# AliaksandrSiarohin/wc-gan

Hardware: AMD Instinct MI355X
Metric: images/sec G+D step, CIFAR-10 ResNet-SN+WC, batch 64 (higher is better)
Workload: dtype f32; 1 GPU; CIFAR-10 ResNet SN uncond + WC (scripts/cifar10_resnet_sn_uncond.sh), batch 64/GPU, training_ratio 5, generator_batch_multiple 2; parallelism=dp1, wc_statistics=per-replica, launch=hipgraph

## Files before the change

wc_gan_amd/csrc/wc_conv.hip:

```cpp
#include "wc_common.h"
#include "../../include/wc_hip.h"
#include <stdlib.h>
#include <string.h>


namespace {

constexpr int kMaxTaps = 16, kMaxPhase = 4;

struct ConvArgs {
    const _Float16* xhi; const _Float16* xlo;
    const _Float16* zero;
    const char* wimg;
    const float* xscale; const float* wscale;
    const float* bias;
    float* y;
    int N, H, W, Hin, Win, Cin, Cout, in_stride, ntaps, nphase, Hout, Wout, out_stride, relu;
    unsigned magHW, shHW, magW, shW;
    int ksplit; float* partial;
    signed char dy[kMaxPhase][kMaxTaps], dx[kMaxPhase][kMaxTaps];
    signed char offy[kMaxPhase], offx[kMaxPhase];
};

__device__ __forceinline__ void lds_dma16(const void* g, unsigned lds)
{
    unsigned keep;
    asm volatile("s_mov_b32 %0, m0\n\ts_mov_b32 m0, %2\n\ts_nop 0\n\tglobal_load_lds_dwordx4 %1, off\n\ts_mov_b32 m0, %0"
                 : "=&s"(keep) : "v"(g), "s"(lds) : "memory");
}

template <int MB, int NB, bool KS>
__device__ __forceinline__ void conv_f16x3_body(const ConvArgs& a, const unsigned bx, const unsigned by, const unsigned bz)
{
    extern __shared__ __attribute__((aligned(16))) char smem[];
    constexpr int TM = 64 * MB, TN = 64 * NB;
    constexpr int A_BYTES = 2 * MB * 4 * 1024, B_BYTES = 2 * NB * 4 * 1024, STAGE = A_BYTES + B_BYTES;
    constexpr int AQ = (2 * MB) / 4;
    static_assert(AQ >= 1, "MB >= 2");

    const int tid = threadIdx.x, lane = tid & 63;
    const int wave = __builtin_amdgcn_readfirstlane(tid >> 6);
    const int wm = wave >> 1, wn = wave & 1;
    const int ntn = a.Cout / TN;
    const int phase = by / ntn, nt = by - phase * ntn;
    const unsigned m0 = bx * TM;
    const unsigned HW = a.H * a.W;
    const int koff = (lane >> 5) * 8;

    int gy[AQ], gx[AQ];
    unsigned gpix[AQ];
    #pragma unroll
    for (int q = 0; q < AQ; ++q) {
        const unsigned m = m0 + (wave * AQ + q) * 32 + (lane & 31);
        const unsigned n = __umulhi(m, a.magHW) >> a.shHW, rem = m - n * HW;
        const unsigned yy = __umulhi(rem, a.magW) >> a.shW, xx = rem - yy * a.W;
        gy[q] = yy * a.in_stride; gx[q] = xx * a.in_stride; gpix[q] = n * (a.Hin * a.Win);
    }
    const unsigned lds0 = (unsigned)(size_t)((__attribute__((address_space(3))) char*)smem);
    const int nchunk = a.Cin >> 5;
    const int iters = a.ntaps * nchunk;
    const int nblk_all = a.Cout >> 5;

    auto issue = [&](int it, int stage) {
        const int tap = it / nchunk, ch = it - tap * nchunk;
        const int dy = a.dy[phase][tap], dx = a.dx[phase][tap];
        const unsigned sbase = __builtin_amdgcn_readfirstlane(lds0 + stage * STAGE);
        #pragma unroll
        for (int q = 0; q < AQ; ++q) {
            const int iy = gy[q] + dy, ix = gx[q] + dx;
            const bool ok = (unsigned)iy < (unsigned)a.Hin && (unsigned)ix < (unsigned)a.Win;
            const int64_t e = ((int64_t)(gpix[q] + iy * a.Win + ix)) * a.Cin + ch * 32 + koff;
            #pragma unroll
            for (int s = 0; s < 2; ++s) {
                const _Float16* ph = ok ? a.xhi + e + s * 16 : a.zero + koff;
                const _Float16* pl = ok ? a.xlo + e + s * 16 : a.zero + koff;
                const unsigned l = sbase + (((wave * AQ + q) * 2 + s) * 2) * 1024;
                lds_dma16(ph, l);
                lds_dma16(pl, l + 1024);
            }
        }
        const char* wsrc = a.wimg + ((((int64_t)(phase * a.ntaps + tap) * nchunk + ch) * nblk_all + nt * 2 * NB) << 12);
        #pragma unroll
        for (int c = 0; c < 2 * NB; ++c) {
            const int idx = wave * 2 * NB + c;
            lds_dma16(wsrc + idx * 1024 + lane * 16, sbase + A_BYTES + idx * 1024);
        }
    };

    f32x16 acc[MB][NB];
    #pragma unroll
    for (int i = 0; i < MB; ++i)
        #pragma unroll
        for (int j = 0; j < NB; ++j)
            #pragma unroll
            for (int r = 0; r < 16; ++r) acc[i][j][r] = 0.f;

    const int it0 = KS ? (int)bz * iters / a.ksplit : 0, it1 = KS ? ((int)bz + 1) * iters / a.ksplit : iters;
    constexpr int NA = AQ * 4, ND = NA + 2 * NB, HALF = ND / 2, PER = 3 * MB * NB, GAP = PER / HALF;
    static_assert(PER % HALF == 0, "DMAs spread evenly");
    int tabv = 0;
    if (lane < a.ntaps) tabv = (a.dy[phase][lane] & 0xff) | ((a.dx[phase][lane] & 0xff) << 8);
    const char* pa[AQ][2];
    int pstep[AQ];
    const char* pw;
    unsigned sb_next = 0;
    auto prep = [&](int it, int stage) {
        const int tap = it / nchunk, ch = it - tap * nchunk;
        const int p = __builtin_amdgcn_readlane(tabv, tap);
        const int dy = (signed char)(p & 0xff), dx = (signed char)((p >> 8) & 0xff);
        #pragma unroll
        for (int q = 0; q < AQ; ++q) {
            const int iy = gy[q] + dy, ix = gx[q] + dx;
            const bool ok = (unsigned)iy < (unsigned)a.Hin && (unsigned)ix < (unsigned)a.Win;
            const int64_t e = ((int64_t)(gpix[q] + iy * a.Win + ix)) * a.Cin + ch * 32 + koff;
            pa[q][0] = reinterpret_cast<const char*>(ok ? a.xhi + e : a.zero + koff);
            pa[q][1] = reinterpret_cast<const char*>(ok ? a.xlo + e : a.zero + koff);
            pstep[q] = ok ? 32 : 0;
        }
        pw = a.wimg + ((((int64_t)(phase * a.ntaps + tap) * nchunk + ch) * nblk_all + nt * 2 * NB) << 12) + wave * (2 * NB * 1024) + lane * 16;
        sb_next = __builtin_amdgcn_readfirstlane(lds0 + stage * STAGE);
    };
    auto dma = [&](int d) {
        if (d < NA) {
            const int q = d >> 2, ks = (d >> 1) & 1, pl = d & 1;
            lds_dma16(pa[q][pl] + ks * pstep[q], sb_next + (((wave * AQ + q) * 2 + ks) * 2 + pl) * 1024);
        } else {
            const int c = d - NA;
            lds_dma16(pw + c * 1024, sb_next + A_BYTES + (wave * 2 * NB + c) * 1024);
        }
    };
    f16x8 fa[2][MB][2], fb[2][NB][2];
    auto frags = [&](int stage, int ks) {
        const char* sa = smem + stage * STAGE;
        const char* sb = sa + A_BYTES;
        #pragma unroll
        for (int i = 0; i < MB; ++i) {
            const char* p = sa + (((wm * MB + i) * 2 + ks) * 2) * 1024 + lane * 16;
            fa[ks][i][0] = *reinterpret_cast<const f16x8*>(p);
            fa[ks][i][1] = *reinterpret_cast<const f16x8*>(p + 1024);
        }
        #pragma unroll
        for (int j = 0; j < NB; ++j) {
            const char* p = sb + (((wn * NB + j) * 2 + ks) * 2) * 1024 + lane * 16;
            fb[ks][j][0] = *reinterpret_cast<const f16x8*>(p);
            fb[ks][j][1] = *reinterpret_cast<const f16x8*>(p + 1024);
        }
    };
    prep(it0, 0);
    #pragma unroll
    for (int d = 0; d < ND; ++d) dma(d);
    for (int it = it0; it < it1; ++it) {
        const int stage = (it - it0) & 1;
        __builtin_amdgcn_s_waitcnt(0x0F70);
        __syncthreads();
        frags(stage, 0);
        prep(it + 1 < it1 ? it + 1 : it, stage ^ 1);
        __builtin_amdgcn_sched_barrier(0);
        #pragma unroll
        for (int ks = 0; ks < 2; ++ks) {
            #pragma unroll
            for (int g = 0; g < PER; ++g) {
                const int prod = g / (MB * NB), i = (g / NB) % MB, j = g % NB;
                acc[i][j] = __builtin_amdgcn_mfma_f32_32x32x16_f16(fa[ks][i][prod == 0 ? 1 : 0], fb[ks][j][prod == 1 ? 1 : 0], acc[i][j], 0, 0, 0);
                if ((g + 1) % GAP == 0) {
                    dma(ks * HALF + g / GAP);
                    __builtin_amdgcn_sched_barrier(0);
                }
                if (ks == 0 && g == PER / 2) {
                    frags(stage, 1);
                    __builtin_amdgcn_sched_barrier(0);
                }
            }
        }
    }
    __builtin_amdgcn_s_waitcnt(0x0F70);
    const float inv = 1.0f / (a.xscale[0] * a.wscale[0]);
    const int oy0 = a.offy[phase], ox0 = a.offx[phase];
    float bj[NB];
    #pragma unroll
    for (int j = 0; j < NB; ++j) bj[j] = a.bias ? a.bias[nt * TN + (wn * NB + j) * 32 + (lane & 31)] : 0.f;
    #pragma unroll
    for (int i = 0; i < MB; ++i) {
        #pragma unroll
        for (int r = 0; r < 16; ++r) {
            const unsigned row = (r & 3) + 8 * (r >> 2) + 4 * (lane >> 5);
            const unsigned m = m0 + (wm * MB + i) * 32 + row;
            const unsigned n = __umulhi(m, a.magHW) >> a.shHW, rem = m - n * HW;
            const unsigned yy = __umulhi(rem, a.magW) >> a.shW, xx = rem - yy * a.W;
            const int64_t opix = ((int64_t)n * a.Hout + (yy * a.out_stride + oy0)) * a.Wout + (xx * a.out_stride + ox0);
            const int64_t oe = opix * a.Cout + nt * TN + wn * NB * 32 + (lane & 31);
            if (KS) {
                float* o = a.partial + (int64_t)bz * ((int64_t)a.N * a.Hout * a.Wout * a.Cout) + oe;
                #pragma unroll
                for (int j = 0; j < NB; ++j) o[j * 32] = acc[i][j][r];
            } else {
                float* o = a.y + oe;
                #pragma unroll
                for (int j = 0; j < NB; ++j) {
                    float v = acc[i][j][r] * inv + bj[j];
                    if (a.relu) v = fmaxf(v, 0.f);
                    o[j * 32] = v;
                }
            }
        }
    }
}

template <int MB, int NB, bool KS>
__global__ __launch_bounds__(256) void conv_f16x3_kernel(ConvArgs a) { conv_f16x3_body<MB, NB, KS>(a, blockIdx.x, blockIdx.y, blockIdx.z); }

struct KsplitReduceArgs {
    const float* partial; int ksplit; int64_t n4; int cout;
    const float* xscale; const float* wscale; const float* bias; int relu; float* y;
};

__device__ __forceinline__ void conv_ksplit_reduce_body(const float* __restrict__ partial, int ksplit, int64_t n4, int cout,
                                                        const float* __restrict__ xscale, const float* __restrict__ wscale,
                                                        const float* __restrict__ bias, int relu, float* __restrict__ y,
                                                        const unsigned bid, const unsigned nblocks, const float* __restrict__ res = nullptr)
{
    const float inv = 1.0f / (xscale[0] * wscale[0]);
    for (int64_t i = (int64_t)bid * 256 + threadIdx.x; i < n4; i += (int64_t)nblocks * 256) {
        f32x4 v = *reinterpret_cast<const f32x4*>(partial + 4 * i);
        int z = 1;
        for (; z + 3 < ksplit; z += 4) {
            f32x4 t[4];
            #pragma unroll
            for (int u = 0; u < 4; ++u) t[u] = *reinterpret_cast<const f32x4*>(partial + 4 * ((z + u) * n4 + i));
            #pragma unroll
            for (int u = 0; u < 4; ++u) v += t[u];
        }
        for (; z < ksplit; ++z) v += *reinterpret_cast<const f32x4*>(partial + 4 * (z * n4 + i));
        v = v * inv;
        if (bias) v += *reinterpret_cast<const f32x4*>(bias + (4 * i) % cout);
        if (relu) { v[0] = fmaxf(v[0], 0.f); v[1] = fmaxf(v[1], 0.f); v[2] = fmaxf(v[2], 0.f); v[3] = fmaxf(v[3], 0.f); }
        if (res) {
            const f32x4 r = *reinterpret_cast<const f32x4*>(res + 4 * i);
            #pragma unroll
            for (int j = 0; j < 4; ++j) v[j] = __fadd_rn(v[j], r[j]);
        }
        *reinterpret_cast<f32x4*>(y + 4 * i) = v;
    }
}

__global__ __launch_bounds__(256) void conv_ksplit_reduce_kernel(const float* __restrict__ partial, int ksplit, int64_t n4, int cout,
                                                                 const float* __restrict__ xscale, const float* __restrict__ wscale,
                                                                 const float* __restrict__ bias, int relu, float* __restrict__ y)
{
    conv_ksplit_reduce_body(partial, ksplit, n4, cout, xscale, wscale, bias, relu, y, blockIdx.x, gridDim.x);
}

__global__ __launch_bounds__(256) void conv_ksplit_reduce_res_kernel(const float* __restrict__ partial, int ksplit, int64_t n4, int cout,
                                                                     const float* __restrict__ xscale, const float* __restrict__ wscale,
                                                                     const float* __restrict__ bias, const float* __restrict__ res,
                                                                     float* __restrict__ y)
{
    conv_ksplit_reduce_body(partial, ksplit, n4, cout, xscale, wscale, bias, 0, y, blockIdx.x, gridDim.x, res);
}

__device__ __forceinline__ f32x4 split_act(f32x4 v, int relu, float slope)
{
    if (relu == 1) { v[0] = fmaxf(v[0], 0.f); v[1] = fmaxf(v[1], 0.f); v[2] = fmaxf(v[2], 0.f); v[3] = fmaxf(v[3], 0.f); }
    else if (relu == 2) {
        #pragma unroll
        for (int j = 0; j < 4; ++j) v[j] = v[j] > 0.f ? v[j] : slope * v[j];
    }
    return v;
}

constexpr int kAmaxBlocks = 512;

__global__ __launch_bounds__(256) void conv_absmax_kernel(const float* __restrict__ x, int64_t n4, int64_t n, float* __restrict__ partial,
                                                          float* __restrict__ colsum = nullptr, int c4n = 0, float leaky = -1.f)
{
    __shared__ float red[4];
    __shared__ f32x4 red4[256];
    float m = 0.f;
    f32x4 cs = {0.f, 0.f, 0.f, 0.f};
    for (int64_t i = blockIdx.x * 256 + threadIdx.x; i < n4; i += (int64_t)gridDim.x * 256) {
        const f32x4 v = *reinterpret_cast<const f32x4*>(x + 4 * i);
        const f32x4 u = leaky >= 0.f ? split_act(v, 2, leaky) : v;
        m = fmaxf(fmaxf(m, fabsf(u[0])), fmaxf(fabsf(u[1]), fmaxf(fabsf(u[2]), fabsf(u[3]))));
        cs += v;
    }
    if (blockIdx.x == 0 && threadIdx.x == 0) for (int64_t i = 4 * n4; i < n; ++i) m = fmaxf(m, fabsf(x[i]));
    #pragma unroll
    for (int o = 32; o > 0; o >>= 1) m = fmaxf(m, __shfl_xor(m, o));
    if ((threadIdx.x & 63) == 0) red[threadIdx.x >> 6] = m;
    if (colsum) red4[threadIdx.x] = cs;
    __syncthreads();
    if (threadIdx.x == 0) partial[blockIdx.x] = fmaxf(fmaxf(red[0], red[1]), fmaxf(red[2], red[3]));
    if (colsum && (int)threadIdx.x < c4n) {
        f32x4 t = red4[threadIdx.x];
        for (int p = threadIdx.x + c4n; p < 256; p += c4n) t += red4[p];
        *reinterpret_cast<f32x4*>(colsum + (int64_t)blockIdx.x * 4 * c4n + 4 * threadIdx.x) = t;
    }
}

__device__ __forceinline__ float scale_of(const float* __restrict__ partial, float mul = 1.0f, int count = kAmaxBlocks)
{
    float amax = 0.f;
    for (int i = threadIdx.x & 63; i < count; i += 64) amax = fmaxf(amax, partial[i]);
    #pragma unroll
    for (int o = 32; o > 0; o >>= 1) amax = fmaxf(amax, __shfl_xor(amax, o));
    amax *= mul;
    if (!(amax > 0.f) || !(amax < 3.0e38f)) return 1.0f;
    int e;
    (void)frexpf(amax, &e);
    return ldexpf(1.0f, 14 - e);
}

__global__ __launch_bounds__(256) void conv_leaky_bwd_kernel(float* __restrict__ dx, const float* __restrict__ x, int64_t n4, float slope)
{
    for (int64_t i = blockIdx.x * 256 + threadIdx.x; i < n4; i += (int64_t)gridDim.x * 256) {
        f32x4 g = *reinterpret_cast<const f32x4*>(dx + 4 * i);
        const f32x4 v = *reinterpret_cast<const f32x4*>(x + 4 * i);
        #pragma unroll
        for (int j = 0; j < 4; ++j) g[j] = v[j] > 0.f ? g[j] : slope * g[j];
        *reinterpret_cast<f32x4*>(dx + 4 * i) = g;
    }
}

template <bool DOWN>
__global__ __launch_bounds__(256) void conv_block_dx_kernel(const float* __restrict__ dx1, const float* __restrict__ x,
                                                            const float* __restrict__ other, int64_t n4, int c4, int W, int H,
                                                            float* __restrict__ out)
{
    for (int64_t i = (int64_t)blockIdx.x * 256 + threadIdx.x; i < n4; i += (int64_t)gridDim.x * 256) {
// ... 676 lines not shown

__global__ __launch_bounds__(256) void conv_wrw_narrow_reduce_kernel(const float* __restrict__ partial, int nparts, int Cin, int ks, int nrow,
                                                                     float* __restrict__ dw, int64_t sk, int64_t sn, int64_t sr, int64_t ss,
                                                                     float* __restrict__ db, int Cout)
{
    __shared__ float red[8][32];
    const int el = threadIdx.x & 31, pg = threadIdx.x >> 5;
    const int e = blockIdx.x * 32 + el;
    const float* p = partial + (int64_t)blockIdx.y * nparts * 4096 + e;
    float sum = 0.f;
    int z = pg;
    for (; z + 8 * 15 < nparts; z += 8 * 16) {
        float v[16];
#pragma unroll
        for (int u = 0; u < 16; ++u) v[u] = p[(int64_t)(z + 8 * u) * 4096];
#pragma unroll
        for (int u = 0; u < 16; ++u) sum += v[u];
    }
    for (; z < nparts; z += 8) sum += p[(int64_t)z * 4096];
    red[pg][el] = sum;
    __syncthreads();
    if (pg != 0) return;
#pragma unroll
    for (int g = 1; g < 8; ++g) sum += red[g][el];
    const int q = e >> 10, r = (e >> 6) & 15, ln = e & 63;
    const int row = (r & 3) + 8 * (r >> 2) + 4 * (ln >> 5);
    const int o = blockIdx.y * 128 + 4 * (ln & 31) + q;
    if (o >= Cout) return;
    if (row < nrow) {
        const int tap = row / Cin, c = row - tap * Cin;
        dw[c * sk + o * sn + (tap / ks) * sr + (tap % ks) * ss] = sum;
    } else if (row == nrow && db) db[o] = sum;
}

struct NarrowFwdArgs {
    const float* x; const float* w; const float* bias; float* y;
    int N, H, W, Cin, Cout, ks, nrow, relu;
    int64_t sk, sn, sr, ss;
    unsigned magHW, shHW, magW, shW;
    int64_t M; int ntiles, tiles_per_wave;
    signed char tdy[32], tdx[32], tch[32], tr[32], ts[32];
};

constexpr int kNarrowLd = 32 * 2 + 4;
constexpr int kNarrowNQ = 2;
template <int KS>
__global__ __launch_bounds__(256, 2) void conv_fwd_narrow_kernel(NarrowFwdArgs a)
{
    __shared__ __attribute__((aligned(16))) float nf_tile[4 * 32 * kNarrowLd];
    const int tid = threadIdx.x, lane = tid & 63;
    const int wave = __builtin_amdgcn_readfirstlane(tid >> 6);
    const int i = lane & 31, k = lane >> 5;
    const int grp = blockIdx.y;
    __shared__ float nf_w[32][32 * kNarrowNQ];
    __shared__ int nf_tab[32][2];
#pragma unroll
    for (int j = 0; j < 8; ++j) {
        const int m = wave + 4 * j;
        const int kind = m < a.nrow ? 0 : (m == a.nrow ? 1 : 2);
        const int o = grp * (32 * kNarrowNQ) + lane;
        float v = 0.f;
        if (kind == 0) v = a.w[a.tch[m] * a.sk + o * a.sn + a.tr[m] * a.sr + a.ts[m] * a.ss];
        else if (kind == 1) v = a.bias ? a.bias[o] : 0.f;
        nf_w[m][lane] = v;
        if (lane == 0) {
            const int dy = a.tdy[m], dx = a.tdx[m];
            nf_tab[m][0] = (dy & 0xff) | ((dx & 0xff) << 8) | (kind << 16);
            nf_tab[m][1] = (dy * a.W + dx) * a.Cin + a.tch[m];
        }
    }
    __syncthreads();
    int dyx[KS], off[KS]; float bw[KS][kNarrowNQ];
#pragma unroll
    for (int s = 0; s < KS; ++s) {
        const int m = 2 * s + k;
        dyx[s] = nf_tab[m][0];
        off[s] = nf_tab[m][1];
#pragma unroll
        for (int q = 0; q < kNarrowNQ; ++q) bw[s][q] = nf_w[m][q * 32 + i];
    }
    const unsigned HW = (unsigned)(a.H * a.W);
    const int t0 = (blockIdx.x * 4 + wave) * a.tiles_per_wave;
    int t1 = t0 + a.tiles_per_wave;
    if (t1 > a.ntiles) t1 = a.ntiles;
    auto gather = [&](int t, float (&av)[KS]) __attribute__((always_inline)) {
        const int64_t p = (int64_t)t * 32 + i;
        const unsigned pc = (unsigned)(p < a.M ? p : a.M - 1);
        const unsigned n = __umulhi(pc, a.magHW) >> a.shHW, rem = pc - n * HW;
        const unsigned yy = __umulhi(rem, a.magW) >> a.shW, xx = rem - yy * a.W;
        const int pb = (int)pc * a.Cin;
#pragma unroll
        for (int s = 0; s < KS; ++s) {
            const int dy = (signed char)(dyx[s] & 0xff), dx = (signed char)((dyx[s] >> 8) & 0xff), kind = dyx[s] >> 16;
            const bool inb = kind == 0 && (unsigned)((int)yy + dy) < (unsigned)a.H && (unsigned)((int)xx + dx) < (unsigned)a.W;
            const float xv = a.x[inb ? pb + off[s] : 0];
            av[s] = inb ? xv : (kind == 1 ? 1.f : 0.f);
        }
    };
    float av[KS], an[KS];
    if (t0 < t1) gather(t0, av);
    for (int t = t0; t < t1; ++t) {
        if (t + 1 < t1) gather(t + 1, an);
        f32x16 acc[kNarrowNQ];
#pragma unroll
        for (int q = 0; q < kNarrowNQ; ++q)
#pragma unroll
            for (int r = 0; r < 16; ++r) acc[q][r] = 0.f;
#pragma unroll
        for (int s = 0; s < KS; ++s)
#pragma unroll
            for (int q = 0; q < kNarrowNQ; ++q) acc[q] = __builtin_amdgcn_mfma_f32_32x32x2f32(av[s], bw[s][q], acc[q], 0, 0, 0);
        float* tl = nf_tile + wave * (32 * kNarrowLd);
#pragma unroll
        for (int r = 0; r < 16; ++r) {
            const int row = (r & 3) + 8 * (r >> 2) + 4 * k;
#pragma unroll
            for (int q = 0; q < kNarrowNQ; ++q) {
                float v = acc[q][r];
                if (a.relu) v = fmaxf(v, 0.f);
                tl[row * kNarrowLd + q * 32 + i] = v;
            }
        }
        __builtin_amdgcn_s_waitcnt(0xc07f);
#pragma unroll
        for (int j = 0; j < 8; ++j) {
            const int row = 4 * j + (lane >> 4);
            const int64_t pr = (int64_t)t * 32 + row;
            const f32x4 v = *reinterpret_cast<const f32x4*>(tl + row * kNarrowLd + 4 * (lane & 15));
            if (pr < a.M) *reinterpret_cast<f32x4*>(a.y + pr * a.Cout + grp * (32 * kNarrowNQ) + 4 * (lane & 15)) = v;
        }
#pragma unroll
        for (int s = 0; s < KS; ++s) av[s] = an[s];
    }
}

void magic_u31(unsigned d, unsigned* mag, unsigned* sh)
{
    unsigned s = 0;
    while ((1u << s) < d) ++s;
    const unsigned long long num = 1ull << (31 + s);
    *mag = (unsigned)((num + d - 1) / d);
    *sh = s - 1;
}

int grid_for(int64_t work_items)
{
    int64_t g = (work_items + 255) / 256;
    return (int)(g < 1 ? 1 : (g > 2048 ? 2048 : g));
}

template <int MB, int NB, bool KS = false>
hipError_t launch_conv(const ConvArgs& a, hipStream_t st)
{
    constexpr int LDS = 2 * (2 * MB * 4 * 1024 + 2 * NB * 4 * 1024);
    hipError_t e = wc_set_max_lds(reinterpret_cast<const void*>(conv_f16x3_kernel<MB, NB, KS>), LDS);
    if (e != hipSuccess) return e;
    const int64_t M = (int64_t)a.N * a.H * a.W;
    dim3 grid((unsigned)(M / (64 * MB)), (unsigned)(a.nphase * (a.Cout / (64 * NB))), (unsigned)a.ksplit);
    hipLaunchKernelGGL((conv_f16x3_kernel<MB, NB, KS>), grid, dim3(256), LDS, st, a);
    return hipGetLastError();
}

}

extern "C" {

static int split_measured(const float* x, int64_t n, int relu, float slope, void* hi, void* lo, float* scale, void* amax_scratch,
                          float* colsum_partials, int C, hipStream_t st)
{
    if (!x || !hi || !lo || !scale || !amax_scratch || n <= 0 || (n & 3)) return WC_ERR_ARG;
    if (colsum_partials && (C <= 0 || (C & 3) || 256 % (C >> 2) != 0 || n % C != 0)) return WC_ERR_SHAPE;
    hipLaunchKernelGGL(conv_absmax_kernel, dim3(kAmaxBlocks), dim3(256), 0, st, x, n / 4, n, (float*)amax_scratch,
                       colsum_partials, colsum_partials ? C >> 2 : 0, relu == 2 ? slope : -1.f);
    hipLaunchKernelGGL(conv_split_kernel, dim3(grid_for(n / 4)), dim3(256), 0, st, x, n / 4, (const float*)amax_scratch, relu,
                       (_Float16*)hi, (_Float16*)lo, scale, slope);
    return (int)hipGetLastError();
}

static int split_hist(const float* x, int64_t n, int relu, float slope, void* hi, void* lo, float* scale, float* colsum_partials, int C,
                      float* hist, int bootstrap, hipStream_t st)
{
    if (!x || !hi || !lo || !scale || !hist || n <= 0 || (n & 3)) return WC_ERR_ARG;
    if (colsum_partials && (C <= 0 || (C & 3) || 256 % (C >> 2) != 0 || n % C != 0)) return WC_ERR_SHAPE;
    if (bootstrap & 1) {
        hipLaunchKernelGGL(conv_absmax_kernel, dim3(kAmaxBlocks), dim3(256), 0, st, x, n / 4, n, hist, colsum_partials, colsum_partials ? C >> 2 : 0,
                           relu == 2 ? slope : -1.f);
        hipLaunchKernelGGL(conv_split_kernel, dim3(grid_for(n / 4)), dim3(256), 0, st, x, n / 4, (const float*)hist, relu, (_Float16*)hi,
                           (_Float16*)lo, scale, slope);
        hipLaunchKernelGGL(conv_hist_seed_kernel, dim3(1), dim3(kAmaxBlocks), 0, st, hist);
        return (int)hipGetLastError();
    }
    hipLaunchKernelGGL(conv_split_hist_kernel, dim3(kAmaxBlocks), dim3(256), 0, st, x, n / 4, relu, (_Float16*)hi, (_Float16*)lo, scale,
                       hist, colsum_partials, colsum_partials ? C >> 2 : 0, slope);
    if (!(bootstrap & 2)) {
        const unsigned g2 = grid_for(n / 4) < 64u ? grid_for(n / 4) : 64u;
        hipLaunchKernelGGL(conv_split_redo_kernel, dim3(g2), dim3(256), 0, st, x, n / 4, relu, (_Float16*)hi, (_Float16*)lo, scale, hist, slope);
    }
    return (int)hipGetLastError();
}

int wc_conv_split_f32(const float* x, int64_t n, int relu, void* hi, void* lo, float* scale, void* amax_scratch, wc_stream_t stream)
{
    return wc_conv_split_colsum_f32(x, n, relu, hi, lo, scale, amax_scratch, nullptr, 0, stream);
}

int wc_conv_split_colsum_f32(const float* x, int64_t n, int relu, void* hi, void* lo, float* scale, void* amax_scratch,
                             float* colsum_partials, int C, wc_stream_t stream)
{
    return split_measured(x, n, relu ? 1 : 0, 0.f, hi, lo, scale, amax_scratch, colsum_partials, C, (hipStream_t)stream);
}

int wc_conv_split_hist_f32(const float* x, int64_t n, int relu, void* hi, void* lo, float* scale, float* colsum_partials, int C,
                           float* hist, int bootstrap, wc_stream_t stream)
{
    return split_hist(x, n, relu ? 1 : 0, 0.f, hi, lo, scale, colsum_partials, C, hist, bootstrap, (hipStream_t)stream);
}

int wc_conv_split_leaky_f32(const float* x, int64_t n, float negative_slope, void* hi, void* lo, float* scale, void* amax_scratch,
                            float* colsum_partials, int C, wc_stream_t stream)
{
    if (!(negative_slope >= 0.f && negative_slope <= 1.f)) return WC_ERR_ARG;
    return split_measured(x, n, negative_slope == 0.f ? 1 : 2, negative_slope, hi, lo, scale, amax_scratch, colsum_partials, C, (hipStream_t)stream);
}

int wc_conv_split_hist_leaky_f32(const float* x, int64_t n, float negative_slope, void* hi, void* lo, float* scale, float* colsum_partials, int C,
                                 float* hist, int bootstrap, wc_stream_t stream)
{
    if (!(negative_slope >= 0.f && negative_slope <= 1.f)) return WC_ERR_ARG;
    return split_hist(x, n, negative_slope == 0.f ? 1 : 2, negative_slope, hi, lo, scale, colsum_partials, C, hist, bootstrap, (hipStream_t)stream);
}

int wc_conv_leaky_bwd_f32(float* dx, const float* x, int64_t n, float negative_slope, wc_stream_t stream)
{
    if (!dx || !x || n <= 0 || (n & 3)) return WC_ERR_ARG;
    hipLaunchKernelGGL(conv_leaky_bwd_kernel, dim3(grid_for(n / 4)), dim3(256), 0, (hipStream_t)stream, dx, x, n / 4, negative_slope);
    return (int)hipGetLastError();
}

size_t wc_conv_weights_bytes(const wc_conv_geom* g)
{
    if (!g) return 0;
    return (size_t)g->nphase * g->ntaps * g->Cin * g->Cout * 4;
}

static int fill_weight_args(WeightArgs& a, const float* w, int64_t stride_k, int64_t stride_n, int64_t stride_r, int64_t stride_s,
                            int64_t n_elems, const wc_conv_geom* g, void* image, float* scale, const float* amax, int amax_count)
{
    if (g->ntaps < 1 || g->ntaps > kMaxTaps || g->nphase < 1 || g->nphase > kMaxPhase || (g->Cin & 31) || (g->Cout & 31)) return WC_ERR_ARG;
    a.w = w; a.sk = stride_k; a.sn = stride_n; a.sr = stride_r; a.ss = stride_s;
    a.amax = amax; a.amax_count = amax_count; a.scale_out = scale; a.img = (char*)image;
    a.n4 = n_elems / 4;
    a.K = g->Cin; a.Nn = g->Cout; a.ntaps = g->ntaps; a.nphase = g->nphase;
    int most = 1;
    for (int p = 0; p < kMaxPhase; ++p)
        for (int t = 0; t < kMaxTaps; ++t) {
            a.nsrc[p][t] = g->nsrc[p][t];
            if (p < g->nphase && t < g->ntaps) {
                if (g->nsrc[p][t] < 1 || g->nsrc[p][t] > 4) return WC_ERR_ARG;
                if (g->nsrc[p][t] > most) most = g->nsrc[p][t];
            }
            for (int m = 0; m < 4; ++m) { a.r[p][t][m] = g->wr[p][t][m]; a.s[p][t][m] = g->ws[p][t][m]; }
        }
    a.coef = g->wcoef; a.bound_mul = fabsf(g->wcoef) * most;
    return WC_OK;
}

int wc_conv_weights_f32(const float* w, int64_t stride_k, int64_t stride_n, int64_t stride_r, int64_t stride_s, int64_t n_elems,
                        const wc_conv_geom* g, void* image, float* scale, void* amax_scratch,
                        const float* known_amax, int known_count, wc_stream_t stream)
{
    hipStream_t st = (hipStream_t)stream;
    if (!w || !g || !image || !scale || (!amax_scratch && !known_amax) || n_elems <= 0) return WC_ERR_ARG;
    if (known_amax && (known_count < 1 || known_count > 4096)) return WC_ERR_ARG;
    const bool inline_max = !known_amax && n_elems <= 32768 && (n_elems & 3) == 0 && ((uintptr_t)w & 15) == 0;
    if (!inline_max && !known_amax) hipLaunchKernelGGL(conv_absmax_kernel, dim3(kAmaxBlocks), dim3(256), 0, st, w, n_elems / 4, n_elems, (float*)amax_scratch);
    WeightArgs a;
    const int rc = fill_weight_args(a, w, stride_k, stride_n, stride_r, stride_s, n_elems, g, image, scale,
                                    inline_max ? nullptr : (known_amax ? known_amax : (const float*)amax_scratch), known_amax ? known_count : kAmaxBlocks);
    if (rc != WC_OK) return rc;
    const int64_t groups = (int64_t)g->nphase * g->ntaps * (g->Cin >> 5) * (g->Cout >> 5) * 128;
    hipLaunchKernelGGL(conv_weights_kernel, dim3(grid_for(groups)), dim3(256), 0, st, a);
    return (int)hipGetLastError();
}

int wc_conv_weights_pair_f32(const float* w, int64_t stride_r, int64_t stride_s, int64_t n_elems,
                             int64_t a_stride_k, int64_t a_stride_n, const wc_conv_geom* ga, void* image_a,
                             int64_t b_stride_k, int64_t b_stride_n, const wc_conv_geom* gb, void* image_b,
                             float* scale, void* amax_scratch, const float* known_amax, int known_count, wc_stream_t stream)
{
    hipStream_t st = (hipStream_t)stream;
    if (!w || !ga || !gb || !image_a || !image_b || !scale || (!amax_scratch && !known_amax) || n_elems <= 0) return WC_ERR_ARG;
    if (known_amax && (known_count < 1 || known_count > 4096)) return WC_ERR_ARG;
    if (!known_amax) hipLaunchKernelGGL(conv_absmax_kernel, dim3(kAmaxBlocks), dim3(256), 0, st, w, n_elems / 4, n_elems, (float*)amax_scratch);
    const float* amax = known_amax ? known_amax : (const float*)amax_scratch;
    const int cnt = known_amax ? known_count : kAmaxBlocks;
    WeightArgs a, b;
    int rc = fill_weight_args(a, w, a_stride_k, a_stride_n, stride_r, stride_s, n_elems, ga, image_a, scale, amax, cnt);
    if (rc != WC_OK) return rc;
    rc = fill_weight_args(b, w, b_stride_k, b_stride_n, stride_r, stride_s, n_elems, gb, image_b, scale + 1, amax, cnt);
    if (rc != WC_OK) return rc;
    if (a.bound_mul != b.bound_mul) return WC_ERR_ARG;
    const int blocks_a = grid_for((int64_t)ga->nphase * ga->ntaps * (ga->Cin >> 5) * (ga->Cout >> 5) * 128);
    const int blocks_b = grid_for((int64_t)gb->nphase * gb->ntaps * (gb->Cin >> 5) * (gb->Cout >> 5) * 128);
    hipLaunchKernelGGL(conv_weights_pair_kernel, dim3(blocks_a + blocks_b), dim3(256), 0, st, a, b, blocks_a);
    return (int)hipGetLastError();
}

// ... 364 lines not shown
    if (!xhi || !xlo || !xscale || !ghi || !glo || !gscale || !zero_line || !g || !dw || !ws) return WC_ERR_NULL;
    if (!wc_conv_supported(g) || (g->Cin & 63) || g->W < 2 || g->H * g->W < 2) return WC_ERR_SHAPE;
    if (ws_bytes < wc_conv_wrw_workspace_bytes(g)) return WC_ERR_WORKSPACE;
    if ((colsum_partials == nullptr) != (db == nullptr)) return WC_ERR_NULL;
    if (db && ((g->Cout & 3) || 256 % (g->Cout >> 2) != 0)) return WC_ERR_SHAPE;
    WrwArgs& a = p.a;
    WrwReduceArgs& r = p.r;
    int T;
    int splits = wrw_splits(g, &T);
    const int64_t M = (int64_t)g->N * g->H * g->W;
    const int nslice = g->nphase * g->ntaps;
    const int tiles = nslice * (g->Cin / T) * (g->Cout / T);
    const int nchunks = (int)(M / 32);
    WrwOperand X, G;
    X.hi = (const _Float16*)xhi; X.lo = (const _Float16*)xlo; X.Hp = g->Hin; X.Wp = g->Win; X.C = g->Cin; X.stride = g->in_stride;
    G.hi = (const _Float16*)ghi; G.lo = (const _Float16*)glo; G.Hp = g->Hout; G.Wp = g->Wout; G.C = g->Cout; G.stride = g->out_stride;
    r.nout = 0; r.coef = g->wcoef;
    for (int ph = 0; ph < kMaxPhase; ++ph)
        for (int t = 0; t < kMaxTaps; ++t) {
            X.dy[ph][t] = g->dy[ph][t]; X.dx[ph][t] = g->dx[ph][t];
            G.dy[ph][t] = g->off_y[ph]; G.dx[ph][t] = g->off_x[ph];
            if (ph >= g->nphase || t >= g->ntaps) continue;
            if (g->nsrc[ph][t] < 1 || g->nsrc[ph][t] > 4) return WC_ERR_ARG;
            for (int m = 0; m < g->nsrc[ph][t]; ++m) {
                int o = 0;
                while (o < r.nout && (r.r[o] != g->wr[ph][t][m] || r.s[o] != g->ws[ph][t][m])) ++o;
                if (o == r.nout) {
                    if (r.nout == kMaxTaps) return WC_ERR_ARG;
                    r.r[o] = g->wr[ph][t][m]; r.s[o] = g->ws[ph][t][m]; r.cnt[o] = 0; ++r.nout;
                }
                if (r.cnt[o] == 4) return WC_ERR_ARG;
                r.slice[o][r.cnt[o]++] = (signed char)(ph * g->ntaps + t);
            }
        }
    const bool x_cols = stride_k == 1;
    a.A = x_cols ? G : X; a.B = x_cols ? X : G;
    a.zero = (const _Float16*)zero_line; a.partial = (float*)ws;
    a.N = g->N; a.H = g->H; a.W = g->W; a.ntaps = g->ntaps; a.nphase = g->nphase;
    magic_u31((unsigned)(g->H * g->W), &a.magHW, &a.shHW);
    magic_u31((unsigned)g->W, &a.magW, &a.shW);
    a.nchunks = nchunks; a.cps = (nchunks + splits - 1) / splits;
    splits = (nchunks + a.cps - 1) / a.cps;
    r.partial = (const float*)ws; r.splits = splits; r.nslice = nslice; r.Ca = a.A.C; r.Cb = a.B.C;
    r.xscale = xscale; r.gscale = gscale; r.dw = dw;
    r.sa = x_cols ? stride_n : stride_k; r.sb = x_cols ? stride_k : stride_n; r.sr = stride_r; r.ss = stride_s;
    r.colsum = colsum_partials; r.db = db; r.c4n = db ? g->Cout >> 2 : 0;
    r.main_blocks = grid_for((int64_t)r.nout * g->Cin * g->Cout);
    p.T = T; p.splits = splits; p.tiles = tiles; p.extra = db ? (r.c4n * 64 + 255) / 256 : 0;
    return WC_OK;
}

int wc_conv_wrw_bias_f16x3(const void* xhi, const void* xlo, const float* xscale, const void* ghi, const void* glo, const float* gscale,
                           const void* zero_line, const wc_conv_geom* g, float* dw, int64_t stride_k, int64_t stride_n,
                           int64_t stride_r, int64_t stride_s, const float* colsum_partials, float* db,
                           void* ws, size_t ws_bytes, wc_stream_t stream)
{
    hipStream_t st = (hipStream_t)stream;
    WrwPlan p;
    const int rc = wrw_prepare(p, xhi, xlo, xscale, ghi, glo, gscale, zero_line, g, dw, stride_k, stride_n, stride_r, stride_s,
                               colsum_partials, db, ws, ws_bytes);
    if (rc != WC_OK) return rc;
    const WrwArgs& a = p.a;
    const WrwReduceArgs& r = p.r;
    const int T = p.T;
    dim3 grid((unsigned)p.splits, (unsigned)p.tiles);
    hipError_t e = hipSuccess;
    if (T == 256) {
        constexpr int LDS = 2 * (2 * 4 * 4 * 1024 + 2 * 4 * 4 * 1024);
        e = wc_set_max_lds(reinterpret_cast<const void*>(conv_wrw_kernel<4, 4>), LDS);
        if (e != hipSuccess) return (int)e;
        hipLaunchKernelGGL((conv_wrw_kernel<4, 4>), grid, dim3(256), LDS, st, a);
    } else if (T == 64) {
        constexpr int LDS = 2 * (2 * 1 * 4 * 1024 + 2 * 1 * 4 * 1024);
        e = wc_set_max_lds(reinterpret_cast<const void*>(conv_wrw_kernel<1, 1>), LDS);
        if (e != hipSuccess) return (int)e;
        hipLaunchKernelGGL((conv_wrw_kernel<1, 1>), grid, dim3(256), LDS, st, a);
    } else {
        constexpr int LDS = 2 * (2 * 2 * 4 * 1024 + 2 * 2 * 4 * 1024);
        e = wc_set_max_lds(reinterpret_cast<const void*>(conv_wrw_kernel<2, 2>), LDS);
        if (e != hipSuccess) return (int)e;
        hipLaunchKernelGGL((conv_wrw_kernel<2, 2>), grid, dim3(256), LDS, st, a);
    }
    hipLaunchKernelGGL(conv_wrw_reduce_kernel, dim3(r.main_blocks + p.extra), dim3(256), 0, st, r);
    return (int)hipGetLastError();
}

int wc_conv_bwd_pair_supported(const wc_conv_geom* gd, const wc_conv_geom* gf)
{
    if (!gd || !gf || !wc_conv_supported(gd) || !wc_conv_supported(gf) || (gf->Cin & 63) || gf->H * gf->W < 2) return 0;
    if (gd->N != gf->N || gd->Cin != gf->Cout || gd->Cout != gf->Cin) return 0;
    if (gd->Hin != gf->Hout || gd->Win != gf->Wout || gd->Hout != gf->Hin || gd->Wout != gf->Win) return 0;
    if (gf->nphase != 1 || gd->in_stride != 1) return 0;
    if ((gd->Cout % 128) != 0 || (gd->Cout % 256) == 0 || conv_big_tile(gd, conv_ksplit(gd))) return 0;
    int tile;
    (void)wrw_splits(gf, &tile);
    return tile == 128 ? 1 : 0;
}

size_t wc_conv_bwd_pair_workspace_bytes(const wc_conv_geom* gd, const wc_conv_geom* gf)
{
    if (!gd || !gf) return 0;
    return wc_conv_workspace_bytes(gd) + wc_conv_wrw_workspace_bytes(gf);
}

int wc_conv_bwd_pair_f16x3(const void* ghi, const void* glo, const float* gscale, const void* wimage, const float* wscale,
                           const void* zero_line, const wc_conv_geom* gd, float* dx, void* ws_dx, size_t ws_dx_bytes,
                           const void* xhi, const void* xlo, const float* xscale, const wc_conv_geom* gf, float* dw,
                           int64_t stride_k, int64_t stride_n, int64_t stride_r, int64_t stride_s,
                           const float* colsum_partials, float* db, void* ws_dw, size_t ws_dw_bytes, wc_stream_t stream)
{
    hipStream_t st = (hipStream_t)stream;
    ConvArgs d;
    int rc = conv_prepare(d, ghi, glo, gscale, wimage, wscale, nullptr, zero_line, gd, 0, dx, ws_dx, ws_dx_bytes);
    if (rc != WC_OK) return rc;
    WrwPlan p;
    rc = wrw_prepare(p, xhi, xlo, xscale, ghi, glo, gscale, zero_line, gf, dw, stride_k, stride_n, stride_r, stride_s,
                     colsum_partials, db, ws_dw, ws_dw_bytes);
    if (rc != WC_OK) return rc;
    if (!wc_conv_bwd_pair_supported(gd, gf) || p.T != 128) return WC_ERR_SHAPE;
    constexpr int LDS = 2 * (2 * 2 * 4 * 1024 + 2 * 2 * 4 * 1024);
    const int64_t M = (int64_t)gd->N * gd->H * gd->W;
    const int gx = (int)(M / 128), gy = gd->nphase * (gd->Cout / 128);
    const int64_t conv_blocks = (int64_t)gx * gy * d.ksplit, wrw_off = (conv_blocks + 7) & ~(int64_t)7;
    const int64_t blocks = wrw_off + (int64_t)p.splits * p.tiles;
    if (blocks > 0x7fffffff) return WC_ERR_SHAPE;
    hipError_t e;
    if (d.ksplit > 1) {
        e = wc_set_max_lds(reinterpret_cast<const void*>(conv_bwd_pair_kernel<true>), LDS);
        if (e != hipSuccess) return (int)e;
        hipLaunchKernelGGL((conv_bwd_pair_kernel<true>), dim3((unsigned)blocks), dim3(256), LDS, st, d, p.a,
                           (int)conv_blocks, (int)wrw_off, p.splits, gx, gy);
    } else {
        e = wc_set_max_lds(reinterpret_cast<const void*>(conv_bwd_pair_kernel<false>), LDS);
        if (e != hipSuccess) return (int)e;
        hipLaunchKernelGGL((conv_bwd_pair_kernel<false>), dim3((unsigned)blocks), dim3(256), LDS, st, d, p.a,
                           (int)conv_blocks, (int)wrw_off, p.splits, gx, gy);
    }
    e = hipGetLastError();
    if (e != hipSuccess) return (int)e;
    const int reduce_blocks = p.r.main_blocks + p.extra;
    if (d.ksplit > 1) {
        KsplitReduceArgs k;
        k.n4 = (int64_t)gd->N * gd->Hout * gd->Wout * gd->Cout / 4;
        k.partial = (const float*)ws_dx; k.ksplit = d.ksplit; k.cout = gd->Cout;
        k.xscale = gscale; k.wscale = wscale; k.bias = nullptr; k.relu = 0; k.y = dx;
        hipLaunchKernelGGL(conv_pair_reduce_kernel, dim3(reduce_blocks + grid_for(k.n4)), dim3(256), 0, st, p.r, k, reduce_blocks);
    } else {
        hipLaunchKernelGGL(conv_wrw_reduce_kernel, dim3(reduce_blocks), dim3(256), 0, st, p.r);
    }
    return (int)hipGetLastError();
}

}
```

Baseline: 3814 images/sec.

## Add half-stage LDS ring pipeline to large-tile f16x3 conv kernel

For tiles with MB*NB>=8, the conv main loop switches from a two-stage double buffer to a ring of half-stage LDS slots. DMAs for the next k-half are spread across the MFMA sequence and each k-half gets a single mid-sequence barrier, which frees fragment reads and address computation from the full-stage sync. The m0 register is set without save/restore, so these loads cost fewer scalar instructions. Optional s_memtime instrumentation, compiled in only under a flag, is added for timing. The scheduling is fragile and depends on the vmcnt arithmetic being exact.

```diff
diff --git a/wc_gan_amd/csrc/wc_conv.hip b/wc_gan_amd/csrc/wc_conv.hip
--- a/wc_gan_amd/csrc/wc_conv.hip
+++ b/wc_gan_amd/csrc/wc_conv.hip
@@ -22,11 +22,51 @@
     signed char offy[kMaxPhase], offx[kMaxPhase];
 };
 
+constexpr bool conv_ring(int MB, int NB)
+{
+#ifdef WC_CONV_RING_OFF
+    return false;
+#else
+    return MB * NB >= 8;
+#endif
+}
+
+#ifdef WC_CONV_STAMPS
+constexpr int kStampTrips = 24, kStampPoints = 6, kStampBytes = 4 * kStampTrips * kStampPoints * 8;
+__device__ unsigned long long wc_conv_stamp_buf[4 * kStampTrips * kStampPoints];
+#define WC_STAMP_DECL                                                                                                              \
+    const bool stamp_wg = MB == 4 && NB == 4 && !KS && (bx | by | bz) == 0;                                                        \
+    unsigned long long* const stamp_lds = reinterpret_cast<unsigned long long*>(smem + 2 * STAGE) + wave * (kStampTrips * kStampPoints); \
+    if (stamp_wg) for (int i = lane; i < kStampTrips * kStampPoints; i += 64) stamp_lds[i] = 0;
+#define WC_STAMP(p)                                                                                                                \
+    if (stamp_wg && it - it0 < kStampTrips) {                                                                                      \
+        const unsigned long long t_ = __builtin_amdgcn_s_memtime();                                                                \
+        if (lane == 0) stamp_lds[(it - it0) * kStampPoints + (p)] = t_;                                                            \
+        __builtin_amdgcn_sched_barrier(0);                                                                                         \
+    }
+#define WC_STAMP_DUMP                                                                                                              \
+    if (stamp_wg) {                                                                                                                \
+        __syncthreads();                                                                                                           \
+        for (int i = tid; i < 4 * kStampTrips * kStampPoints; i += 256)                                                            \
+            wc_conv_stamp_buf[i] = reinterpret_cast<const unsigned long long*>(smem + 2 * STAGE)[i];                               \
+    }
+#else
+constexpr int kStampBytes = 0;
+#define WC_STAMP_DECL
+#define WC_STAMP(p)
+#define WC_STAMP_DUMP
+#endif
+
 __device__ __forceinline__ void lds_dma16(const void* g, unsigned lds)
 {
     unsigned keep;
     asm volatile("s_mov_b32 %0, m0\n\ts_mov_b32 m0, %2\n\ts_nop 0\n\tglobal_load_lds_dwordx4 %1, off\n\ts_mov_b32 m0, %0"
                  : "=&s"(keep) : "v"(g), "s"(lds) : "memory");
+}
+
+__device__ __forceinline__ void lds_dma16_m0(const void* g, unsigned lds)
+{
+    asm volatile("s_mov_b32 m0, %1\n\ts_nop 0\n\tglobal_load_lds_dwordx4 %0, off" : : "v"(g), "s"(lds) : "memory", "m0");
 }
 
 template <int MB, int NB, bool KS>
@@ -146,13 +186,125 @@
             fb[ks][j][1] = *reinterpret_cast<const f16x8*>(p + 1024);
         }
     };
+    WC_STAMP_DECL
+    if constexpr (conv_ring(MB, NB)) {
+    constexpr int NPRE = (PER / 4 - 1) / GAP + 1, G0 = PER / 4 + (MB + NB), REST = HALF - NPRE, STEP = (PER - (AQ + 1) - G0) / REST;
+    static_assert(NPRE >= 1 && REST >= 1 && STEP >= 1 && (NPRE - 1) * GAP < PER / 4, "both runs of DMAs have room");
+    auto dma_at = [](int g) {
+        if (g < G0) return (g % GAP == 0 && g / GAP < NPRE) ? g / GAP : -1;
+        return ((g - G0) % STEP == 0 && (g - G0) / STEP < REST) ? NPRE + (g - G0) / STEP : -1;
+    };
+    constexpr int SLOT = STAGE / 2, A_HALF = A_BYTES / 2, BAR = PER / 4, AHEAD = HALF + NPRE, PIECES = AQ + 1, NF = 2 * (MB + NB);
+    static_assert(NB % 2 == 0, "a wave stages whole n-blocks");
+    static_assert(G0 + (REST - 1) * STEP < PER - PIECES, "the address pieces stand behind the k-step's last DMA");
+    static_assert(AHEAD > 0 && AHEAD < 64 && 2 * HALF < 64, "vmcnt is six bits");
+    int ntap = it0 / nchunk, nch = it0 - ntap * nchunk, nleft = it1 - it0 - 1;
+    int pdy = 0, pdx = 0;
+    auto piece = [&](int p) {
+        if (p == 0) {
+            const int t = __builtin_amdgcn_readlane(tabv, ntap);
+            pdy = (signed char)(t & 0xff); pdx = (signed char)((t >> 8) & 0xff);
+        }
+        if (p < AQ) {
+            const int iy = gy[p] + pdy, ix = gx[p] + pdx;
+            const bool ok = (unsigned)iy < (unsigned)a.Hin && (unsigned)ix < (unsigned)a.Win;
+            const int64_t e = ((int64_t)(gpix[p] + iy * a.Win + ix)) * a.Cin + nch * 32 + koff;
+            pa[p][0] = reinterpret_cast<const char*>(ok ? a.xhi + e : a.zero + koff);
+            pa[p][1] = reinterpret_cast<const char*>(ok ? a.xlo + e : a.zero + koff);
+            pstep[p] = ok ? 32 : 0;
+        } else {
+            pw = a.wimg + ((((int64_t)(phase * a.ntaps + ntap) * nchunk + nch) * nblk_all + nt * 2 * NB) << 12) + wave * (2 * NB * 1024) + lane * 16;
+        }
+    };
+    auto advance = [&]() {
+        if (nleft > 0) {
+            --nleft;
+            if (++nch == nchunk) { nch = 0; ++ntap; }
+        }
+    };
+    auto rdma = [&](int d, int ks, unsigned slot) {
+        if (d < 2 * AQ) {
+            const int q = d >> 1, pl = d & 1;
+            lds_dma16_m0(pa[q][pl] + ks * pstep[q], slot + ((wave * AQ + q) * 2 + pl) * 1024);
+        } else {
+            const int c = d - 2 * AQ, jj = c >> 1, pl = c & 1;
+            lds_dma16_m0(pw + ((jj * 2 + ks) * 2 + pl) * 1024, slot + A_HALF + ((wave * (NB / 2) + jj) * 2 + pl) * 1024);
+        }
+    };
+    auto rfrag = [&](int slot, int set, int n) {
+        const char* sa = smem + slot * SLOT + lane * 16;
+        if (n < 2 * MB) fa[set][n >> 1][n & 1] = *reinterpret_cast<const f16x8*>(sa + ((wm * MB + (n >> 1)) * 2 + (n & 1)) * 1024);
+        else            fb[set][(n >> 1) - MB][n & 1] = *reinterpret_cast<const f16x8*>(sa + A_HALF + ((wn * NB + (n >> 1) - MB) * 2 + (n & 1)) * 1024);
+    };
+    #pragma unroll
+    for (int p = 0; p < PIECES; ++p) piece(p);
+    #pragma unroll
+    for (int d = 0; d < HALF; ++d) rdma(d, 0, lds0);
+    #pragma unroll
+    for (int d = 0; d < HALF; ++d) rdma(d, 1, lds0 + SLOT);
+    advance();
+    #pragma unroll
+    for (int p = 0; p < PIECES; ++p) piece(p);
+    #pragma unroll
+    for (int d = 0; d < HALF; ++d) rdma(d, 0, lds0 + 2 * SLOT);
+    asm volatile("s_waitcnt vmcnt(%0)" :: "n"(2 * HALF) : "memory");
+    __builtin_amdgcn_s_barrier();
+    asm volatile("" ::: "memory");
+    #pragma unroll
+    for (int n = 0; n < NF; ++n) rfrag(0, 0, n);
+    __builtin_amdgcn_sched_barrier(0);
+    int s0 = 0;
+    for (int it = it0; it < it1; ++it) {
+        WC_STAMP(0)
+        #pragma unroll
+        for (int h = 0; h < 2; ++h) {
+            const unsigned dst = __builtin_amdgcn_readfirstlane(lds0 + (h == 0 ? (s0 ^ 2) + 1 : s0) * SLOT);
+            const int pub = h == 0 ? s0 + 1 : s0 ^ 2;
+            #pragma unroll
+            for (int g = 0; g < PER; ++g) {
+                const int prod = g / (MB * NB), i = (g / NB) % MB, j = g % NB;
+                acc[i][j] = __builtin_amdgcn_mfma_f32_32x32x16_f16(fa[h][i][prod == 0 ? 1 : 0], fb[h][j][prod == 1 ? 1 : 0], acc[i][j], 0, 0, 0);
+                if (dma_at(g) >= 0) {
+                    __builtin_amdgcn_sched_barrier(0);
+                    rdma(dma_at(g), h ^ 1, dst);
+                    __builtin_amdgcn_sched_barrier(0);
+                }
+                if (g == BAR) {
+                    __builtin_amdgcn_sched_barrier(0);
+                    asm volatile("s_waitcnt vmcnt(%0) lgkmcnt(0)" :: "n"(AHEAD) : "memory");
+                    WC_STAMP(1 + 2 * h)
+                    __builtin_amdgcn_s_barrier();
+                    asm volatile("" ::: "memory");
+                    WC_STAMP(2 + 2 * h)
+                }
+                if (g >= BAR && g < G0) {
+                    rfrag(pub, h ^ 1, 2 * (g - BAR));
+                    rfrag(pub, h ^ 1, 2 * (g - BAR) + 1);
+                    __builtin_amdgcn_sched_barrier(0);
+                }
+                if (h == 0 && g >= PER - PIECES) {
+                    if (g == PER - PIECES) advance();
+                    piece(g - (PER - PIECES));
+                    __builtin_amdgcn_sched_barrier(0);
+                }
+            }
+        }
+        s0 ^= 2;
+        WC_STAMP(5)
+    }
+    __builtin_amdgcn_s_waitcnt(0x0F70);
+    WC_STAMP_DUMP
+    } else {
     prep(it0, 0);
     #pragma unroll
     for (int d = 0; d < ND; ++d) dma(d);
     for (int it = it0; it < it1; ++it) {
         const int stage = (it - it0) & 1;
+        WC_STAMP(0)
         __builtin_amdgcn_s_waitcnt(0x0F70);
+        WC_STAMP(1)
         __syncthreads();
+        WC_STAMP(2)
         frags(stage, 0);
         prep(it + 1 < it1 ? it + 1 : it, stage ^ 1);
         __builtin_amdgcn_sched_barrier(0);
@@ -170,10 +322,14 @@
                     frags(stage, 1);
                     __builtin_amdgcn_sched_barrier(0);
                 }
+                if (ks == 0 && g == 0) { WC_STAMP(3) }
             }
         }
+        WC_STAMP(5)
     }
     __builtin_amdgcn_s_waitcnt(0x0F70);
+    WC_STAMP_DUMP
+    }
     const float inv = 1.0f / (a.xscale[0] * a.wscale[0]);
     const int oy0 = a.offy[phase], ox0 = a.offx[phase];
     float bj[NB];
@@ -1156,7 +1312,7 @@
 template <int MB, int NB, bool KS = false>
 hipError_t launch_conv(const ConvArgs& a, hipStream_t st)
 {
-    constexpr int LDS = 2 * (2 * MB * 4 * 1024 + 2 * NB * 4 * 1024);
+    constexpr int LDS = 2 * (2 * MB * 4 * 1024 + 2 * NB * 4 * 1024) + kStampBytes;
     hipError_t e = wc_set_max_lds(reinterpret_cast<const void*>(conv_f16x3_kernel<MB, NB, KS>), LDS);
     if (e != hipSuccess) return e;
     const int64_t M = (int64_t)a.N * a.H * a.W;
@@ -1827,3 +1983,12 @@
 }
 
 }
+
+#ifdef WC_CONV_STAMPS
+extern "C" int wc_conv_stamps_read(unsigned long long* dst, int* trips, int* points)
+{
+    if (!dst || !trips || !points) return WC_ERR_ARG;
+    *trips = kStampTrips; *points = kStampPoints;
+    return (int)hipMemcpyFromSymbol(dst, HIP_SYMBOL(wc_conv_stamp_buf), sizeof(wc_conv_stamp_buf), 0, hipMemcpyDeviceToHost);
+}
+#endif
```

After: 3811 images/sec. No clear change (-0.1%).
